# ZechengLi19/CIM

Measured on AMD Instinct MI355X. Metric: images/sec training step (ResNet-50 VOC, ~1k proposals/img) at 1/2/4/8 GPU, higher is better.
Workload: dtype fp32

## Files before the change

cim_amd/csrc/conv1x1.hip:

```cpp
#include "common.h"
#include "../../include/cim_hip.h"

#ifndef CIM_BODY_PRIO_LEVEL
#define CIM_BODY_PRIO_LEVEL 3
#endif
#if CIM_BODY_PRIO_LEVEL > 0
#define CIM_BODY_PRIO() __builtin_amdgcn_s_setprio(CIM_BODY_PRIO_LEVEL)
#else
#define CIM_BODY_PRIO()
#endif
namespace {

#ifndef CIM_SMALL_BK
#define CIM_SMALL_BK 32
#endif
#ifndef CIM_SMALL_ABL
#define CIM_SMALL_ABL 0
#endif
constexpr int SBM = 64, SBN = 64, SBK = CIM_SMALL_BK;
constexpr int SLD = 68;
typedef float f32x16 __attribute__((ext_vector_type(16)));
typedef float f32x4u __attribute__((ext_vector_type(4), aligned(4)));
__device__ __forceinline__ float4 ld4(const float* p) {
    const f32x4u v = *reinterpret_cast<const f32x4u*>(p);
// ... 193 lines not shown
#define SM_GLOAD(RA, RB, S)                                                                                        \
    {                                                                                                              \
        _Pragma("unroll") for (int i = 0; i < PA; ++i) asm volatile("" : "+v"(RA[i].x), "+v"(RA[i].y), "+v"(RA[i].z), "+v"(RA[i].w)); \
        _Pragma("unroll") for (int i = 0; i < PB; ++i) asm volatile("" : "+v"(RB[i].x), "+v"(RB[i].y), "+v"(RB[i].z), "+v"(RB[i].w)); \
    }
#else
#define SM_GLOAD(RA, RB, S)                                                                                        \
    {                                                                                                              \
        _Pragma("unroll") for (int i = 0; i < PA; ++i) RA[i] = bld4(RA_, oa[i] + (unsigned)(S) * sa);               \
        _Pragma("unroll") for (int i = 0; i < PB; ++i) RB[i] = bld4(RB_, ob[i] + (unsigned)(S) * sb);               \
    }
#endif
#define SM_PUT(RA, RB, BUF, S)                                                                                     \
    {                                                                                                              \
        _Pragma("unroll") for (int i = 0; i < PA; ++i)                                                             \
            tile_store<AM, SBM>(As[BUF], tile_ktail<AM, SBM>(RA[i], g.K, kbeg + (S) * SBK, tid + i * NT), tid + i * NT);     \
        _Pragma("unroll") for (int i = 0; i < PB; ++i)                                                             \
            tile_store<!BKc, BNT>(Bs[BUF], tile_ktail<!BKc, BNT>(RB[i], g.K, kbeg + (S) * SBK, tid + i * NT), tid + i * NT); \
    }
#define SM_MMA(BUF)                                                                                                \
    {                                                                                                              \
        const float* __restrict__ a = As[BUF] + (lane >> 5) * SLD + wm * 32 + (lane & 31);                         \
        const float* __restrict__ b = Bs[BUF] + (lane >> 5) * SLD + wn * 32 + (lane & 31);                         \
        float av[SBK / 2], bv[SBK / 2];                                                                            \
        _Pragma("unroll") for (int t = 0; t < SBK / 2; ++t) { av[t] = a[2 * t * SLD]; bv[t] = b[2 * t * SLD]; }    \
        _Pragma("unroll") for (int t = 0; t < (CIM_SMALL_ABL == 1 ? 1 : SBK / 2); ++t)                             \
            acc = __builtin_amdgcn_mfma_f32_32x32x2f32(av[t], bv[t], acc, 0, 0, 0);                                \
        asm volatile("" : "+a"(acc));       \
    }
    if (kbeg < kend) {
        const int nslab = (kend - kbeg + SBK - 1) / SBK;
        const int last = nslab - 1;
        SM_GLOAD(ra0, rb0, 0)
        SM_GLOAD(ra1, rb1, min(1, last))
        SM_PUT(ra0, rb0, 0, 0)
        asm volatile("" : "+a"(acc));
        __syncthreads();
        for (int s = 0; s < nslab; s += 2) {
            SM_GLOAD(ra0, rb0, min(s + 2, last))
            SM_MMA(0)
            if (s + 1 < nslab) SM_PUT(ra1, rb1, 1, s + 1)
            __syncthreads();
            if (s + 1 >= nslab) break;
            SM_GLOAD(ra1, rb1, min(s + 3, last))
            SM_MMA(1)
            if (s + 2 < nslab) SM_PUT(ra0, rb0, 0, s + 2)
            __syncthreads();
        }
    }
#undef SM_GLOAD
#undef SM_PUT
#undef SM_MMA

    small_epilogue(g, acc, m0 + wm * 32, n0 + wn * 32, lane, split, ColIdentity{g.N});
}

__device__ __forceinline__ float splitk_sum(const float* __restrict__ ws, size_t i, size_t mn, int splits) {
    float v = ws[i];
    for (int k0 = 1; k0 < splits; k0 += 8) {
        float p[8];
#pragma unroll
        for (int j = 0; j < 8; ++j) p[j] = k0 + j < splits ? ws[(size_t)(k0 + j) * mn + i] : 0.0f;
#pragma unroll
        for (int j = 0; j < 8; ++j)
            if (k0 + j < splits) v += p[j];
    }
    return v;
}
__global__ __launch_bounds__(256) void small_splitk_reduce_kernel(const SmallArgs g) {
    CIM_BODY_PRIO();
    const size_t i = (size_t)blockIdx.x * 256 + threadIdx.x;
    const size_t mn = (size_t)g.M * g.N;
    if (i >= mn) return;
    small_finish(g, (int)(i / g.N), (int)(i % g.N), splitk_sum(g.ws, i, mn, g.splits));
}
__global__ __launch_bounds__(256) void small_splitk_reduce4_kernel(const SmallArgs g) {
    CIM_BODY_PRIO();
    const size_t q = (size_t)blockIdx.x * 256 + threadIdx.x;
    const size_t mn = (size_t)g.M * g.N;
    const size_t i = q * 4;
    if (i >= mn) return;
    float4 v = *reinterpret_cast<const float4*>(g.ws + i);
    for (int k0 = 1; k0 < g.splits; k0 += 4) {
        float4 p[4];
#pragma unroll
        for (int j = 0; j < 4; ++j)
            p[j] = k0 + j < g.splits ? *reinterpret_cast<const float4*>(g.ws + (size_t)(k0 + j) * mn + i) : make_float4(0.f, 0.f, 0.f, 0.f);
#pragma unroll
        for (int j = 0; j < 4; ++j)
            if (k0 + j < g.splits) { v.x += p[j].x; v.y += p[j].y; v.z += p[j].z; v.w += p[j].w; }
    }
    int row = (int)(i / g.N), col = (int)(i - (size_t)row * g.N);
    const float s[4] = {v.x, v.y, v.z, v.w};
    float y[4], s1 = 0.0f, s2 = 0.0f;
#pragma unroll
    for (int j = 0; j < 4; ++j) {
        y[j] = small_value(g, row, col, s[j], s1, s2);
        if (++col == g.N) { col = 0; ++row; }
    }
    if (g.Xraw) *reinterpret_cast<float4*>(g.Xraw + i) = v;
    *reinterpret_cast<float4*>(g.C + i) = make_float4(y[0], y[1], y[2], y[3]);
}

__global__ __launch_bounds__(256) void small_splitk_reduce_rows_kernel(const SmallArgs g) {
    CIM_BODY_PRIO();
    const int col = blockIdx.x * 256 + threadIdx.x, row = blockIdx.y;
    const size_t mn = (size_t)g.M * g.N;
    float s1 = 0.0f, s2 = 0.0f;
    if (col < g.N) {
        const size_t i = (size_t)row * g.N + col;
        small_finish(g, row, col, splitk_sum(g.ws, i, mn, g.splits), s1, s2);
    }
    small_put_part(g, row, col >> 5, threadIdx.x & 63, s1, s2);
}

struct BnPartTable { cim_bn_part_desc d[24]; int first[25]; int n; };
__global__ __launch_bounds__(256) void bn_part_finish_kernel(const BnPartTable t) {
    CIM_BODY_PRIO();
    __shared__ float sh[2][8][32];
    int e = 0;
    while (e + 1 < t.n && (int)blockIdx.x >= t.first[e + 1]) ++e;
    const cim_bn_part_desc& d = t.d[e];
    const int C = d.channels, parts = d.parts, total = d.images * d.parts;
    const int c = ((int)blockIdx.x - t.first[e]) * 32 + (threadIdx.x & 31), grp = threadIdx.x >> 5;
    float t1 = 0.0f, t2 = 0.0f;
    if (c < C) {
        for (int i0 = grp; i0 < total; i0 += 32) {
            float a[4], b[4];
#pragma unroll
            for (int j = 0; j < 4; ++j) {
                const int i = i0 + 8 * j;
                const int img = i / parts, p = i - img * parts;
                const float* q = d.part + ((size_t)img * 2 * parts + p) * C + c;
                a[j] = i < total ? q[0] : 0.0f;
                b[j] = i < total ? q[(size_t)parts * C] : 0.0f;
            }
#pragma unroll
            for (int j = 0; j < 4; ++j) { t1 += a[j]; t2 += b[j]; }
        }
    }
    sh[0][grp][threadIdx.x & 31] = t1;
    sh[1][grp][threadIdx.x & 31] = t2;
    __syncthreads();
    if (grp == 0 && c < C) {
        float a1 = 0.0f, a2 = 0.0f;
#pragma unroll
        for (int k = 0; k < 8; ++k) { a1 += sh[0][k][threadIdx.x]; a2 += sh[1][k][threadIdx.x]; }
        if (d.dbeta) d.dbeta[c] = a1;
        if (d.dgamma) d.dgamma[c] = a2 * rsqrtf(d.var[c] + d.eps);
    }
}

enum { CONV_FWD = 0, CONV_DX = 1, CONV_DW = 2 };
struct ConvGeom { int H, W, Ho, Wo, stride, cin, cout; float inv_w; int dil; };

#ifndef CIM_CONV3_BK
#define CIM_CONV3_BK 32
#endif
constexpr int CBK = CIM_CONV3_BK;
template <int MODE, int KS = 3>
__global__ __launch_bounds__(256) void conv3x3_small_kernel(const SmallArgs g, const ConvGeom c) {
    CIM_BODY_PRIO();
    constexpr int TAPS = KS * KS;
    constexpr int NT = 256, PA = SBM * (CBK / 4) / NT, PB = SBN * (CBK / 4) / NT;
    extern __shared__ __attribute__((aligned(16))) float c3_smem[];
    float (*As)[CBK * SLD] = reinterpret_cast<float (*)[CBK * SLD]>(c3_smem);
    float (*Bs)[CBK * SLD] = reinterpret_cast<float (*)[CBK * SLD]>(c3_smem + 2 * CBK * SLD);
    const int tid = threadIdx.x, lane = tid & 63, wave = tid >> 6;
    const int wm = wave >> 1, wn = wave & 1;
    const int tiles_n = (g.N + SBN - 1) / SBN;
    const int m0 = (blockIdx.x / tiles_n) * SBM, n0 = (blockIdx.x % tiles_n) * SBN;
    const int split = blockIdx.y;
    const int kper = ((g.K + g.splits - 1) / g.splits + CBK - 1) / CBK * CBK;
    const int kbeg = split * kper, kend = min(g.K, kbeg + kper);

    const rsrc_t RA_ = make_rsrc(g.A, tile_extent(MODE == CONV_DX, g.M, g.K, g.lda));
    const rsrc_t RB_ = make_rsrc(g.B, (long long)(MODE == CONV_DX ? c.cout * c.Ho * c.Wo : c.cin * c.H * c.W));
    const int hw_src = MODE == CONV_DX ? c.Ho * c.Wo : c.H * c.W;
    int py[PB][4], px[PB][4];
    int boff[PB], bdy[PB], bdx[PB];
#pragma unroll
    for (int i = 0; i < PB; ++i) {
        const int p = tid + i * NT;
        if (MODE == CONV_DW) {
            const int n = n0 + p % SBN;
            const int ch = n / TAPS, tap = n - ch * TAPS;
            boff[i] = n < g.N ? ch * hw_src : -1;
            bdy[i] = (tap / KS - KS / 2) * c.dil;
            bdx[i] = (tap - (tap / KS) * KS - KS / 2) * c.dil;
        } else {
            const int wrow = (MODE == CONV_DX) ? c.W : c.Wo;
#pragma unroll
            for (int j = 0; j < 4; ++j) {
                const int n = n0 + (p % 16) * 4 + j;
                const int y = (int)(((float)n + 0.5f) * c.inv_w);
                py[i][j] = n < g.N ? y : -(1 << 20);
                px[i][j] = n - y * wrow;
            }
        }
    }
    unsigned oa[PA];
#pragma unroll
    for (int i = 0; i < PA; ++i) oa[i] = tile_off<MODE == CONV_DX, SBM>(g.lda, m0, kbeg, tid + i * NT);
    const unsigned sa = (MODE == CONV_DX ? (unsigned)g.lda * CBK : (unsigned)CBK) * 4u;

    auto load_b = [&](int k0, float4 (&rb)[PB]) {
#pragma unroll
        for (int i = 0; i < PB; ++i) {
            const int p = tid + i * NT;
            unsigned off[4];
            if (MODE == CONV_DW) {
                const int k = k0 + (p / SBN) * 4;
#pragma unroll
                for (int j = 0; j < 4; ++j) {
                    const int po = k + j;
                    const int yo = (int)(((float)po + 0.5f) * c.inv_w), xo = po - yo * c.Wo;
                    const int yi = yo * c.stride + bdy[i], xi = xo * c.stride + bdx[i];
                    const bool ok = boff[i] >= 0 && po < g.K && (unsigned)yi < (unsigned)c.H && (unsigned)xi < (unsigned)c.W;
                    off[j] = ok ? (unsigned)(boff[i] + yi * c.W + xi) * 4u : OOB;
                }
            } else {
                const int k = k0 + p / 16;
                const int ch = k / TAPS, tap = k - ch * TAPS;
                const int dy = (tap / KS - KS / 2) * c.dil, dx = (tap - (tap / KS) * KS - KS / 2) * c.dil;
                const int base = ch * hw_src;
#pragma unroll
                for (int j = 0; j < 4; ++j) {
                    if (MODE == CONV_DX) {
                        const int ty = py[i][j] - dy, tx = px[i][j] - dx;
                        const int yo = c.stride == 2 ? ty >> 1 : ty, xo = c.stride == 2 ? tx >> 1 : tx;
                        const bool ok = ty >= 0 && tx >= 0 && yo < c.Ho && xo < c.Wo && !(c.stride == 2 && ((ty | tx) & 1));
                        off[j] = ok ? (unsigned)(base + yo * c.Wo + xo) * 4u : OOB;
                    } else {
                        const int yi = py[i][j] * c.stride + dy, xi = px[i][j] * c.stride + dx;
                        const bool ok = (unsigned)yi < (unsigned)c.H && (unsigned)xi < (unsigned)c.W;
                        off[j] = ok ? (unsigned)(base + yi * c.W + xi) * 4u : OOB;
                    }
                }
            }
#if CIM_SMALL_ABL == 3
            asm volatile("" : "+v"(rb[i].x), "+v"(rb[i].y), "+v"(rb[i].z), "+v"(rb[i].w) : "v"(off[0]), "v"(off[1]), "v"(off[2]), "v"(off[3]));
#elif CIM_SMALL_ABL == 5
            rb[i] = make_float4(bld1(RB_, (unsigned)(p * 16 + k0 * 64)), bld1(RB_, (unsigned)(p * 16 + k0 * 64 + 4)),
                                bld1(RB_, (unsigned)(p * 16 + k0 * 64 + 8)), bld1(RB_, (unsigned)(p * 16 + k0 * 64 + 12)));
#else
            rb[i] = make_float4(bld1(RB_, off[0]), bld1(RB_, off[1]), bld1(RB_, off[2]), bld1(RB_, off[3]));
#endif
        }
    };
    auto load_a = [&](int s, float4 (&ra)[PA]) {
#pragma unroll
        for (int i = 0; i < PA; ++i)
            ra[i] = bld4(RA_, oa[i] + (unsigned)s * sa);
    };

    f32x16 acc;
#pragma unroll
    for (int i = 0; i < 16; ++i) acc[i] = 0.0f;
    float4 ra0[PA], rb0[PB], ra1[PA], rb1[PB];
#define C3_PUT(RA, RB, BUF, S)                                                                                      \
    {                                                                                                               \
        _Pragma("unroll") for (int i = 0; i < PA; ++i)                                                              \
            tile_store<MODE == CONV_DX, SBM>(As[BUF], tile_ktail<MODE == CONV_DX, SBM>(RA[i], g.K, kbeg + (S) * CBK, tid + i * NT), tid + i * NT); \
        _Pragma("unroll") for (int i = 0; i < PB; ++i) tile_store<MODE != CONV_DW, SBN>(Bs[BUF], RB[i], tid + i * NT); \
    }
#define C3_MMA(BUF)                                                                                                 \
    {                                                                                                               \
        const float* __restrict__ a = As[BUF] + (lane >> 5) * SLD + wm * 32 + (lane & 31);                          \
        const float* __restrict__ b = Bs[BUF] + (lane >> 5) * SLD + wn * 32 + (lane & 31);                          \
        float av[CBK / 2], bv[CBK / 2];                                                                             \
        _Pragma("unroll") for (int t = 0; t < CBK / 2; ++t) { av[t] = a[2 * t * SLD]; bv[t] = b[2 * t * SLD]; }     \
        _Pragma("unroll") for (int t = 0; t < (CIM_SMALL_ABL == 1 ? 1 : CBK / 2); ++t)                              \
            acc = __builtin_amdgcn_mfma_f32_32x32x2f32(av[t], bv[t], acc, 0, 0, 0);                                 \
        asm volatile("" : "+a"(acc));                                                                               \
    }
    if (kbeg < kend) {
        const int nslab = (kend - kbeg + CBK - 1) / CBK;
        const int last = nslab - 1;
        load_a(0, ra0); load_b(kbeg, rb0);
        load_a(min(1, last), ra1); load_b(kbeg + min(1, last) * CBK, rb1);
        C3_PUT(ra0, rb0, 0, 0)
        asm volatile("" : "+a"(acc));
        __syncthreads();
        for (int s = 0; s < nslab; s += 2) {
            load_a(min(s + 2, last), ra0); load_b(kbeg + min(s + 2, last) * CBK, rb0);
            C3_MMA(0)
            if (s + 1 < nslab) C3_PUT(ra1, rb1, 1, s + 1)
            __syncthreads();
            if (s + 1 >= nslab) break;
            load_a(min(s + 3, last), ra1); load_b(kbeg + min(s + 3, last) * CBK, rb1);
            C3_MMA(1)
            if (s + 2 < nslab) C3_PUT(ra0, rb0, 0, s + 2)
            __syncthreads();
        }
    }
#undef C3_PUT
#undef C3_MMA
    small_epilogue(g, acc, m0 + wm * 32, n0 + wn * 32, lane, split, ColIdentity{g.N});
}

struct Dx2Geom { int H, W, Ho, Wo, cin, cout; int first[5]; int tiles_n[4]; int group0[4]; };

__global__ __launch_bounds__(256) void conv3x3_dx2_kernel(const SmallArgs g, const Dx2Geom c) {
    CIM_BODY_PRIO();
    constexpr int NT = 256, PA = SBM * (CBK / 4) / NT, PB = SBN * (CBK / 4) / NT;
    extern __shared__ __attribute__((aligned(16))) float d2_smem[];
    float (*As)[CBK * SLD] = reinterpret_cast<float (*)[CBK * SLD]>(d2_smem);
    float (*Bs)[CBK * SLD] = reinterpret_cast<float (*)[CBK * SLD]>(d2_smem + 2 * CBK * SLD);
    const int tid = threadIdx.x, lane = tid & 63, wave = tid >> 6;
    const int wm = wave >> 1, wn = wave & 1;
    int cls = 0;
    while (cls < 3 && (int)blockIdx.x >= c.first[cls + 1]) ++cls;
    const int py = cls >> 1, px = cls & 1;
    const int Wc = (c.W - px + 1) >> 1, Nc = ((c.H - py + 1) >> 1) * Wc;
    const int local = (int)blockIdx.x - c.first[cls], tn = c.tiles_n[cls];
    const int m0 = (local / tn) * SBM, n0 = (local % tn) * SBN;
    const int nx = px ? 2 : 1, lgT = py + px, T = 1 << lgT;
    const int K = c.cout << lgT;
    const int nslab = (K + CBK - 1) / CBK;
    const int how = c.Ho * c.Wo;
    const rsrc_t RA_ = make_rsrc(g.A, tile_extent(true, g.M, 9 * c.cout, g.lda));
    const rsrc_t RB_ = make_rsrc(g.B, (long long)c.cout * how);
    int yc[PB][4], xc[PB][4];
#pragma unroll
    for (int i = 0; i < PB; ++i) {
        const int p = tid + i * NT;
#pragma unroll
        for (int j = 0; j < 4; ++j) {
            const int nc = n0 + (p % 16) * 4 + j;
            const int y = nc / Wc;
            yc[i][j] = nc < Nc ? y : -(1 << 20);
            xc[i][j] = nc - y * Wc;
        }
    }
    auto tap_of = [&](int j, int& tap, int& oy, int& ox) {
        const int jy = j / nx, jx = j - jy * nx;
        const int ky = py ? 2 * jy : 1, kx = px ? 2 * jx : 1;
        tap = ky * 3 + kx;
        oy = (py && jy == 0) ? 1 : 0;
        ox = (px && jx == 0) ? 1 : 0;
    };
    auto load_a = [&](int k0, float4 (&ra)[PA]) {
#pragma unroll
        for (int i = 0; i < PA; ++i) {
            const int p = tid + i * NT;
            const int k = k0 + p / (SBM / 4), r = m0 + (p % (SBM / 4)) * 4;
            const int co = k >> lgT;
            int tap, oy, ox;
            tap_of(k & (T - 1), tap, oy, ox);
            ra[i] = bld4(RA_, co < c.cout ? ((unsigned)(co * 9 + tap) * g.lda + r) * 4u : OOB);
        }
    };
    auto load_b = [&](int k0, float4 (&rb)[PB]) {
#pragma unroll
        for (int i = 0; i < PB; ++i) {
            const int p = tid + i * NT;
            const int k = k0 + p / 16;
            const int co = k >> lgT;
            int tap, oy, ox;
            tap_of(k & (T - 1), tap, oy, ox);
            const int base = co * how;
            unsigned off[4];
#pragma unroll
            for (int j = 0; j < 4; ++j) {
                const int yo = yc[i][j] + oy, xo = xc[i][j] + ox;
                const bool ok = co < c.cout && yo >= 0 && yo < c.Ho && xo < c.Wo;
                off[j] = ok ? (unsigned)(base + yo * c.Wo + xo) * 4u : OOB;
            }
            rb[i] = make_float4(bld1(RB_, off[0]), bld1(RB_, off[1]), bld1(RB_, off[2]), bld1(RB_, off[3]));
        }
    };
    f32x16 acc;
#pragma unroll
    for (int i = 0; i < 16; ++i) acc[i] = 0.0f;
    float4 ra0[PA], rb0[PB], ra1[PA], rb1[PB];
#define D2_PUT(RA, RB, BUF)                                                                                         \
    {                                                                                                               \
        _Pragma("unroll") for (int i = 0; i < PA; ++i) tile_store<true, SBM>(As[BUF], RA[i], tid + i * NT);          \
        _Pragma("unroll") for (int i = 0; i < PB; ++i) tile_store<true, SBN>(Bs[BUF], RB[i], tid + i * NT);          \
    }
#define D2_MMA(BUF)                                                                                                 \
    {                                                                                                               \
        const float* __restrict__ a = As[BUF] + (lane >> 5) * SLD + wm * 32 + (lane & 31);                          \
        const float* __restrict__ b = Bs[BUF] + (lane >> 5) * SLD + wn * 32 + (lane & 31);                          \
        float av[CBK / 2], bv[CBK / 2];                                                                             \
        _Pragma("unroll") for (int t = 0; t < CBK / 2; ++t) { av[t] = a[2 * t * SLD]; bv[t] = b[2 * t * SLD]; }     \
        _Pragma("unroll") for (int t = 0; t < CBK / 2; ++t)                                                         \
            acc = __builtin_amdgcn_mfma_f32_32x32x2f32(av[t], bv[t], acc, 0, 0, 0);                                 \
        asm volatile("" : "+a"(acc));                                                                               \
    }
    {
        const int last = nslab - 1;
        load_a(0, ra0); load_b(0, rb0);
        load_a(min(1, last) * CBK, ra1); load_b(min(1, last) * CBK, rb1);
        D2_PUT(ra0, rb0, 0)
        asm volatile("" : "+a"(acc));
        __syncthreads();
        for (int s = 0; s < nslab; s += 2) {
            load_a(min(s + 2, last) * CBK, ra0); load_b(min(s + 2, last) * CBK, rb0);
            D2_MMA(0)
            if (s + 1 < nslab) D2_PUT(ra1, rb1, 1)
            __syncthreads();
            if (s + 1 >= nslab) break;
            load_a(min(s + 3, last) * CBK, ra1); load_b(min(s + 3, last) * CBK, rb1);
            D2_MMA(1)
            if (s + 2 < nslab) D2_PUT(ra0, rb0, 0)
            __syncthreads();
        }
    }
#undef D2_PUT
#undef D2_MMA
    small_epilogue(g, acc, m0 + wm * 32, n0 + wn * 32, lane, 0, ColParity{Wc, c.W, py, px, Nc, c.group0[cls]});
}

__global__ __launch_bounds__(256) void conv3x3_wt_kernel(const float* __restrict__ w, float* __restrict__ wt, int cin) {
    extern __shared__ float wt_s[];
    const int co = blockIdx.x, n = cin * 9;
    for (int i = threadIdx.x; i < n; i += 256) wt_s[i] = w[(size_t)co * n + i];
    __syncthreads();
    for (int i = threadIdx.x; i < n; i += 256) {
        const int tap = i / cin, ci = i - tap * cin;
        wt[(size_t)co * n + i] = wt_s[ci * 9 + tap];
    }
}

struct WtTable { cim_wt_desc d[16]; int first[17]; int n; };
__global__ __launch_bounds__(256) void conv3x3_wt_multi_kernel(const WtTable t) {
    extern __shared__ float wt_s[];
    int e = 0;
    while (e + 1 < t.n && (int)blockIdx.x >= t.first[e + 1]) ++e;
    const int co = blockIdx.x - t.first[e], cin = t.d[e].cin, n = cin * 9;
    const float* __restrict__ w = t.d[e].w;
    float* __restrict__ wt = t.d[e].wt;
    for (int i = threadIdx.x; i < n; i += 256) wt_s[i] = w[(size_t)co * n + i];
    __syncthreads();
    for (int i = threadIdx.x; i < n; i += 256) {
        const int tap = i / cin, ci = i - tap * cin;
        wt[(size_t)co * n + i] = wt_s[ci * 9 + tap];
    }
}

SmallArgs small_args(const float* A, const float* B, float* C, int M, int N, int K, int lda, int ldb, int ldc, int splits, float* ws,
                     const InputBn* in_bn, float* x_raw = nullptr, const float* gamma = nullptr, const float* beta = nullptr,
                     const float* mean = nullptr, const float* var = nullptr, float eps = 0.f, const float* residual = nullptr, int relu = 0) {
    SmallArgs g{};
    g.A = A; g.B = B; g.C = C; g.Xraw = x_raw;
    g.gamma = gamma; g.beta = beta; g.mean = mean; g.var = var; g.res = residual; g.eps = eps;
    g.M = M; g.N = N; g.K = K; g.lda = lda; g.ldb = ldb; g.ldc = ldc;
    g.relu = relu; g.bn = gamma != nullptr;
    g.splits = splits; g.ws = ws;
    if (in_bn) {
        g.mask = in_bn->y; g.mgamma = in_bn->gamma; g.mvar = in_bn->var; g.meps = in_bn->eps;
        g.mxr = in_bn->xr; g.mmean = in_bn->mean; g.mpart = in_bn->part; g.mparts = (N + 31) / 32;
    }
    return g;
}
template <class Kernel, class... Args>
int launch_lds(Kernel kern, dim3 grid, size_t lds, hipStream_t st, const Args&... args) {
    if (lds > 48 * 1024) {
        hipError_t e = hipFuncSetAttribute(reinterpret_cast<const void*>(kern), hipFuncAttributeMaxDynamicSharedMemorySize, (int)lds);
        if (e != hipSuccess) return (int)e;
    }
    hipLaunchKernelGGL(kern, grid, dim3(256), lds, st, args...);
    return 0;
}
static void launch_splitk_reduce(const SmallArgs& g, hipStream_t st) {
    if (g.mpart) {
        hipLaunchKernelGGL(small_splitk_reduce_rows_kernel, dim3((unsigned)((g.N + 255) / 256), (unsigned)g.M), dim3(256), 0, st, g);
    } else {
        const size_t n = (size_t)g.M * g.N;
        if (n >= (1u << 19) && g.ldc == g.N && n % 4 == 0 && (((size_t)g.ws | (size_t)g.C | (size_t)g.Xraw) & 15) == 0)
            hipLaunchKernelGGL(small_splitk_reduce4_kernel, dim3((unsigned)((n / 4 + 255) / 256)), dim3(256), 0, st, g);
        else
            hipLaunchKernelGGL(small_splitk_reduce_kernel, dim3((unsigned)((n + 255) / 256)), dim3(256), 0, st, g);
    }
}

template <bool AM, bool BKc>
static void launch_small(const SmallArgs& g, int splits, hipStream_t st, bool narrow) {
    const long long tm = (g.M + SBM - 1) / SBM;
    if (narrow)
        hipLaunchKernelGGL((gemm_small_kernel<AM, BKc, 1>), dim3((unsigned)(tm * ((g.N + 31) / 32)), (unsigned)splits), dim3(128), 0, st, g);
    else
        hipLaunchKernelGGL((gemm_small_kernel<AM, BKc, 2>), dim3((unsigned)(tm * ((g.N + 63) / 64)), (unsigned)splits), dim3(256), 0, st, g);
}

}

extern "C" int cim_gemm_small_splits(int M, int N, int K) {
    const long long tiles = (long long)((M + SBM - 1) / SBM) * ((N + SBN - 1) / SBN);
#ifndef CIM_SMALL_WGS
#define CIM_SMALL_WGS 512
#endif
#ifndef CIM_SMALL_MINSLABS
#define CIM_SMALL_MINSLABS 4
#endif
    constexpr int min_k = CIM_SMALL_MINSLABS * SBK, want = CIM_SMALL_WGS;
    int s = 1;
    while (tiles * s < want && K / (s * 2) >= min_k && s < 64) s *= 2;
    return s;
}

static int gemm_small_impl(const float* A, const float* B, float* C, int M, int N, int K, int lda, int ldb, int ldc,
                           int a_mcontig, int b_kcontig, float* x_raw, const float* gamma, const float* beta,
                           const float* mean, const float* var, float eps, const float* residual, int relu, int splits,
                           float* workspace, void* stream, const InputBn* in_bn, int res_w = 0) {
    CIM_CHECK_ARG(res_w == 0 || (residual && res_w > 0 && N % res_w == 0 && ldc == N));
    CIM_CHECK_ARG(A && B && C && M > 0 && N > 0 && K > 0 && lda > 0 && ldb > 0 && ldc >= N && splits >= 1);
    CIM_CHECK_ARG((gamma == nullptr) == (beta == nullptr) && (gamma == nullptr) == (mean == nullptr) && (gamma == nullptr) == (var == nullptr));
    CIM_CHECK_ARG(splits == 1 || workspace);
    SmallArgs g = small_args(A, B, C, M, N, K, lda, ldb, ldc, splits, workspace, in_bn, x_raw, gamma, beta, mean, var, eps, residual, relu);
    g.a_mcontig = a_mcontig; g.b_kcontig = b_kcontig;
    g.res_w = res_w;
    if (res_w) { g.res_ws = (res_w + 1) / 2; g.res_hw = ((N / res_w + 1) / 2) * g.res_ws; }
    const long long tiles = (long long)((M + SBM - 1) / SBM) * ((N + SBN - 1) / SBN);
    CIM_CHECK_ARG(tiles * 2 < (1ll << 31) && splits <= 65535 && M <= 65535);
    CIM_CHECK_ARG(tile_extent(a_mcontig != 0, M, K, lda) < (1ll << 29) && tile_extent(b_kcontig == 0, N, K, ldb) < (1ll << 29));
    const bool narrow = tiles * splits < 128;
    hipStream_t st = cim::as_stream(stream);
    if (a_mcontig) {
        if (b_kcontig) launch_small<true, true>(g, splits, st, narrow); else launch_small<true, false>(g, splits, st, narrow);
    } else {
        if (b_kcontig) launch_small<false, true>(g, splits, st, narrow); else launch_small<false, false>(g, splits, st, narrow);
    }
    if (splits > 1) launch_splitk_reduce(g, st);
    CIM_CHECK_LAUNCH();
    return 0;
}

extern "C" int cim_gemm_small_f32(const float* A, const float* B, float* C, int M, int N, int K, int lda, int ldb, int ldc,
                                  int a_mcontig, int b_kcontig, float* x_raw, const float* gamma, const float* beta,
                                  const float* mean, const float* var, float eps, const float* residual, int relu, int splits,
                                  float* workspace, void* stream) {
    return gemm_small_impl(A, B, C, M, N, K, lda, ldb, ldc, a_mcontig, b_kcontig, x_raw, gamma, beta, mean, var, eps, residual, relu,
                           splits, workspace, stream, nullptr);
}

extern "C" int cim_linear_bias_f32(const float* X, const float* W, const float* bias, float* Y, int M, int N, int K, int splits,
                                   float* workspace, void* stream) {
    CIM_CHECK_ARG(X && W && Y && M > 0 && N > 0 && K > 0 && splits >= 1 && splits <= 65535 && (splits == 1 || workspace));
    SmallArgs g = small_args(X, W, Y, M, N, K, K, K, N, splits, workspace, nullptr);
    g.b_kcontig = 1; g.colbias = bias;
    hipStream_t st = cim::as_stream(stream);
    launch_small<false, true>(g, splits, st, false);
    if (splits > 1) {
        const size_t n = (size_t)M * N;
        hipLaunchKernelGGL(small_splitk_reduce_kernel, dim3((unsigned)((n + 255) / 256)), dim3(256), 0, st, g);
    }
    CIM_CHECK_LAUNCH();
    return 0;
}

extern "C" long long cim_conv1x1_bwd_workspace(int B, int cin, int cout, int hw) {
    const long long dx = (long long)cim_gemm_small_splits(cin, hw, cout) * cin * hw;
    const long long dw = (long long)cim_gemm_small_splits(cout, cin, hw) * cout * cin + (B > 1 ? (long long)cout * cin : 0);
    const long long dconv = (long long)B * cout * hw;
    return (long long)sizeof(float) * (dconv + dx + dw);
}

namespace {
struct ForkJoin {
    hipStream_t main, side;
    hipEvent_t ev_fork, ev_join;
    bool on;
    ForkJoin(hipStream_t m, hipStream_t s, void* fork_event, void* join_event, bool want)
        : main(m), side(s), ev_fork(static_cast<hipEvent_t>(fork_event)), ev_join(static_cast<hipEvent_t>(join_event)),
          on(want && s != nullptr && s != m) {}
    hipStream_t fork() {
        if (!on) return main;
        (void)hipEventRecord(ev_fork, main);
        (void)hipStreamWaitEvent(side, ev_fork, 0);
        return side;
    }
    void join() {
        if (!on) return;
        (void)hipEventRecord(ev_join, side);
        (void)hipStreamWaitEvent(main, ev_join, 0);
    }
};

__global__ __launch_bounds__(256) void small_axpy_kernel(float* __restrict__ y, const float* __restrict__ x, size_t n) {
    const size_t i = (size_t)blockIdx.x * 256 + threadIdx.x;
    if (i < n) y[i] += x[i];
}
template <class Product>
int dw_over_images(int B, float* dw, float* ws_dw, int sp, size_t n, hipStream_t st, Product product) {
    for (int b = 0; b < B && dw; ++b) {
        float* out = b == 0 ? dw : ws_dw + (size_t)sp * n;
        const int rc = product(b, out);
        if (rc) return rc;
        if (b) hipLaunchKernelGGL(small_axpy_kernel, dim3((unsigned)((n + 255) / 256)), dim3(256), 0, st, dw, out, n);
    }
    return 0;
}
}

extern "C" int cim_conv1x1_bn_act_bwd(const float* dy, const float* y, const float* x_raw, const float* x, const float* w,
                                      const float* gamma, const float* mean, const float* var, float eps, int relu,
                                      float* dres, float* dgamma, float* dbeta, float* dx, float* dw, int B, int cin, int cout,
                                      int hw, float* workspace, void* stream, void* side_stream, void* fork_event, void* join_event, int join,
                                      int dy_is_dconv, const float* in_gamma, const float* in_var, float in_eps,
                                      const float* in_xr, const float* in_mean, float* in_part, const float* dx_add, int dx_add_w) {
    CIM_CHECK_ARG(dx_add_w == 0 || (dx_add != nullptr && dx_add_w > 0 && hw % dx_add_w == 0));
    CIM_CHECK_ARG(side_stream == nullptr || side_stream == stream || (fork_event != nullptr && (!join || join_event != nullptr)));
    const size_t add_bs = dx_add_w ? (size_t)cin * ((hw / dx_add_w + 1) / 2) * ((dx_add_w + 1) / 2) : (size_t)cin * hw;
    CIM_CHECK_ARG(dy && x_raw && x && w && gamma && mean && var && workspace && B > 0 && cin > 0 && cout > 0 && hw > 0);
    CIM_CHECK_ARG(dx_add == nullptr || (dx != nullptr && in_gamma == nullptr));
    CIM_CHECK_ARG((y != nullptr || !relu) && ((dgamma == nullptr) == (dbeta == nullptr)));
    CIM_CHECK_ARG(!dy_is_dconv || (dres == nullptr && dgamma == nullptr));
    CIM_CHECK_ARG((in_gamma == nullptr) == (in_var == nullptr));
    CIM_CHECK_ARG(in_part == nullptr || (in_gamma && in_xr && in_mean));
    float* dconv = dy_is_dconv ? const_cast<float*>(dy) : workspace;
    float* ws_dx = workspace + (size_t)B * cout * hw;
    float* ws_dw = ws_dx + (size_t)cim_gemm_small_splits(cin, hw, cout) * cin * hw;
    int rc = dy_is_dconv ? 0 : cim_bn_act_bwd(dy, y, x_raw, gamma, mean, var, eps, dconv, dres, dgamma, dbeta, B, cout, hw, relu, stream);
    if (rc) return rc;
    ForkJoin fj(cim::as_stream(stream), cim::as_stream(side_stream), fork_event, join_event, dx && dw);
    hipStream_t st_dw = fj.fork();
    const int sp = cim_gemm_small_splits(cout, cin, hw);
    rc = dw_over_images(B, dw, ws_dw, sp, (size_t)cout * cin, st_dw, [&](int b, float* out) {
        return cim_gemm_small_f32(dconv + (size_t)b * cout * hw, x + (size_t)b * cin * hw, out, cout, cin, hw, hw, hw, cin, 0, 1,
                                  nullptr, nullptr, nullptr, nullptr, nullptr, 0.f, nullptr, 0, sp, ws_dw, st_dw);
    });
    if (rc) return rc;
    for (int b = 0; b < B && dx; ++b) {
        const InputBn ib{x + (size_t)b * cin * hw, in_gamma, in_var, in_eps, in_xr ? in_xr + (size_t)b * cin * hw : nullptr, in_mean,
                         in_part ? in_part + (size_t)b * 2 * ((hw + 31) / 32) * cin : nullptr};
        rc = gemm_small_impl(w, dconv + (size_t)b * cout * hw, dx + (size_t)b * cin * hw, cin, hw, cout, cin, hw, hw, 1, 0,
                             nullptr, nullptr, nullptr, nullptr, nullptr, 0.f, dx_add ? dx_add + (size_t)b * add_bs : nullptr, 0,
                             cim_gemm_small_splits(cin, hw, cout), ws_dx, stream, in_gamma ? &ib : nullptr, dx_add_w);
        if (rc) return rc;
    }
    if (join) fj.join();
    CIM_CHECK_LAUNCH();
    return 0;
}

namespace {
int conv3x3_launch(int mode, const float* A, const float* B, float* C, int M, int N, int K, int lda, int ldc, const ConvGeom& c,
                   float* x_raw, const float* gamma, const float* beta, const float* mean, const float* var, float eps,
                   const float* residual, int relu, int splits, float* ws, hipStream_t st, int ksize = 3, const InputBn* in_bn = nullptr) {
    SmallArgs g = small_args(A, B, C, M, N, K, lda, 0, ldc, splits, ws, in_bn, x_raw, gamma, beta, mean, var, eps, residual, relu);
    g.b_kcontig = mode == CONV_DW;
    const dim3 grid((unsigned)(((M + SBM - 1) / SBM) * ((N + SBN - 1) / SBN)), (unsigned)splits);
    auto kern = ksize == 7 ? conv3x3_small_kernel<CONV_FWD, 7>
                : mode == CONV_FWD ? conv3x3_small_kernel<CONV_FWD> : mode == CONV_DX ? conv3x3_small_kernel<CONV_DX> : conv3x3_small_kernel<CONV_DW>;
    const int rc = launch_lds(kern, grid, sizeof(float) * 4 * CBK * SLD, st, g, c);
    if (rc) return rc;
    if (splits > 1) launch_splitk_reduce(g, st);
    return 0;
}
ConvGeom conv_geom(int cin, int cout, int H, int W, int stride, int mode, int dil = 1) {
    ConvGeom c;
    c.H = H; c.W = W; c.stride = stride; c.cin = cin; c.cout = cout; c.dil = dil;
    c.Ho = (H - 1) / stride + 1; c.Wo = (W - 1) / stride + 1;
    c.inv_w = 1.0f / (float)(mode == CONV_DX ? W : c.Wo);
    return c;
}
}

#define CONV3_ARGS_OK(CIN_MULT)                                                                                      \
    CIM_CHECK_ARG(cin > 0 && cout > 0 && H > 0 && W > 0 && (stride == 1 || stride == 2) && W <= 4096 &&               \
                  dilation >= 1 && dilation <= 8 && (dilation == 1 || stride == 1) &&                                 \
                  (long long)H * W < (1ll << 20) && (long long)cin * H * W < (1ll << 29) && (long long)cout * H * W < (1ll << 29) && \
                  (long long)cin * cout * 9 < (1ll << 29) && cin % (CIN_MULT) == 0)

extern "C" int cim_conv3x3_nchw_splits(int cin, int cout, int H, int W, int stride) {
    const int Ho = (H - 1) / stride + 1, Wo = (W - 1) / stride + 1;
    return cim_gemm_small_splits(cout, Ho * Wo, 9 * cin);
}

extern "C" int cim_conv3x3_nchw_f32(const float* x, const float* w, float* y, int cin, int cout, int H, int W, int stride,
                               int dilation, float* x_raw, const float* gamma, const float* beta, const float* mean, const float* var,
                               float eps, const float* residual, int relu, int splits, float* workspace, void* stream) {
    CIM_CHECK_ARG(x && w && y && splits >= 1 && splits <= 65535 && (splits == 1 || workspace));
    CONV3_ARGS_OK(1);
    CIM_CHECK_ARG((gamma == nullptr) == (beta == nullptr) && (gamma == nullptr) == (mean == nullptr) && (gamma == nullptr) == (var == nullptr));
    const ConvGeom c = conv_geom(cin, cout, H, W, stride, CONV_FWD, dilation);
    conv3x3_launch(CONV_FWD, w, x, y, cout, c.Ho * c.Wo, 9 * cin, 9 * cin, c.Ho * c.Wo, c, x_raw, gamma, beta, mean, var, eps,
                   residual, relu, splits, workspace, cim::as_stream(stream));
    CIM_CHECK_LAUNCH();
    return 0;
}

extern "C" int cim_conv7x7_nchw_f32(const float* x, const float* w, float* y, int cin, int cout, int H, int W, int stride,
                                    const float* gamma, const float* beta, const float* mean, const float* var, float eps,
                                    int relu, void* stream) {
    CIM_CHECK_ARG(x && w && y && cin > 0 && cout > 0 && H > 0 && W > 0 && (stride == 1 || stride == 2) && W <= 4096);
    CIM_CHECK_ARG((long long)H * W < (1ll << 20) && (long long)cin * H * W < (1ll << 29) && (long long)cout * H * W < (1ll << 29));
    CIM_CHECK_ARG((gamma == nullptr) == (beta == nullptr) && (gamma == nullptr) == (mean == nullptr) && (gamma == nullptr) == (var == nullptr));
    const ConvGeom c = conv_geom(cin, cout, H, W, stride, CONV_FWD);
    conv3x3_launch(CONV_FWD, w, x, y, cout, c.Ho * c.Wo, 49 * cin, 49 * cin, c.Ho * c.Wo, c, nullptr, gamma, beta, mean, var, eps,
                   nullptr, relu, 1, nullptr, cim::as_stream(stream), 7);
    CIM_CHECK_LAUNCH();
    return 0;
}

namespace {
Dx2Geom dx2_geom(int cin, int cout, int H, int W) {
    Dx2Geom c{};
    c.H = H; c.W = W; c.Ho = (H - 1) / 2 + 1; c.Wo = (W - 1) / 2 + 1; c.cin = cin; c.cout = cout;
    const int tiles_m = (cin + SBM - 1) / SBM;
    int first = 0, group = 0;
    for (int cls = 0; cls < 4; ++cls) {
        const int py = cls >> 1, px = cls & 1;
        const int nc = ((H - py + 1) / 2) * ((W - px + 1) / 2);
        c.first[cls] = first;
        c.tiles_n[cls] = (nc + SBN - 1) / SBN;
        c.group0[cls] = group;
        first += tiles_m * c.tiles_n[cls];
        group += 2 * c.tiles_n[cls];
    }
    c.first[4] = first;
    return c;
}
}

extern "C" int cim_conv3x3_dx_parts(int H, int W, int stride) {
    if (stride != 2) return (H * W + 31) / 32;
    int parts = 0;
    for (int cls = 0; cls < 4; ++cls) parts += 2 * ((((H - (cls >> 1) + 1) / 2) * ((W - (cls & 1) + 1) / 2) + SBN - 1) / SBN);
    return parts;
}

extern "C" long long cim_conv3x3_nchw_bwd_workspace(int B, int cin, int cout, int H, int W, int stride) {
    const int Ho = (H - 1) / stride + 1, Wo = (W - 1) / stride + 1;
    const long long dx = (long long)cim_gemm_small_splits(cin, H * W, 9 * cout) * cin * H * W;
    const long long dw = (long long)cim_gemm_small_splits(cout, 9 * cin, Ho * Wo) * cout * cin * 9 + (B > 1 ? (long long)cout * cin * 9 : 0);
    const long long dconv = (long long)B * cout * Ho * Wo;
    return (long long)sizeof(float) * (dconv + (long long)cout * cin * 9 + dx + dw);
}

extern "C" int cim_bn_part_finish(const cim_bn_part_desc* descs, int n, void* stream) {
    CIM_CHECK_ARG(descs && n > 0);
    hipStream_t st = cim::as_stream(stream);
    for (int base = 0; base < n; base += 24) {
        BnPartTable t{};
        t.n = n - base < 24 ? n - base : 24;
        int total = 0;
        for (int i = 0; i < t.n; ++i) {
            const cim_bn_part_desc& d = descs[base + i];
            CIM_CHECK_ARG(d.part && d.var && (d.dgamma || d.dbeta) && d.images > 0 && d.parts > 0 && d.channels > 0);
            t.d[i] = d;
            t.first[i] = total;
            total += (d.channels + 31) / 32;
        }
        t.first[t.n] = total;
        hipLaunchKernelGGL(bn_part_finish_kernel, dim3((unsigned)total), dim3(256), 0, st, t);
    }
    CIM_CHECK_LAUNCH();
    return 0;
}

extern "C" int cim_conv3x3_wt_multi(const cim_wt_desc* descs, int n, void* stream) {
    CIM_CHECK_ARG(descs && n > 0);
    hipStream_t st = cim::as_stream(stream);
    for (int base = 0; base < n; base += 16) {
        WtTable t{};
        t.n = n - base < 16 ? n - base : 16;
        int total = 0, max_cin = 0;
        for (int i = 0; i < t.n; ++i) {
            const cim_wt_desc& d = descs[base + i];
            CIM_CHECK_ARG(d.w && d.wt && d.cin > 0 && d.cout > 0 && (size_t)d.cin * 9 * sizeof(float) <= 64 * 1024);
            t.d[i] = d;
            t.first[i] = total;
            total += d.cout;
            max_cin = d.cin > max_cin ? d.cin : max_cin;
        }
        t.first[t.n] = total;
        const int rc = launch_lds(conv3x3_wt_multi_kernel, dim3((unsigned)total), sizeof(float) * max_cin * 9, st, t);
        if (rc) return rc;
    }
    CIM_CHECK_LAUNCH();
    return 0;
}

extern "C" int cim_conv3x3_nchw_bn_act_bwd(const float* dy, const float* y, const float* x_raw, const float* x, const float* w,
                                      const float* gamma, const float* mean, const float* var, float eps, int relu,
                                      float* dres, float* dgamma, float* dbeta, float* dx, float* dw, int B, int cin, int cout,
                                      int H, int W, int stride, int dilation, float* workspace, void* stream, void* side_stream,
                                      void* fork_event, void* join_event, int join, int dy_is_dconv, const float* in_gamma, const float* in_var, float in_eps,
                                      const float* in_xr, const float* in_mean, float* in_part, const float* wt_ready) {
    CIM_CHECK_ARG(dy && x_raw && x && w && gamma && mean && var && workspace && B > 0);
    CIM_CHECK_ARG(side_stream == nullptr || side_stream == stream || (fork_event != nullptr && (!join || join_event != nullptr)));
    CONV3_ARGS_OK(4);
    CIM_CHECK_ARG((y != nullptr || !relu) && ((dgamma == nullptr) == (dbeta == nullptr)) && cout % 4 == 0);
    CIM_CHECK_ARG(!dy_is_dconv || (dres == nullptr && dgamma == nullptr));
    CIM_CHECK_ARG((in_gamma == nullptr) == (in_var == nullptr));
    CIM_CHECK_ARG(in_part == nullptr || (in_gamma && in_xr && in_mean));
    const ConvGeom cx = conv_geom(cin, cout, H, W, stride, CONV_DX, dilation), cw = conv_geom(cin, cout, H, W, stride, CONV_DW, dilation);
    const int hwo = cx.Ho * cx.Wo, hw = H * W;
    hipStream_t st = cim::as_stream(stream);
    float* dconv = dy_is_dconv ? const_cast<float*>(dy) : workspace;
    float* wt_own = workspace + (size_t)B * cout * hwo;
    const float* wt = wt_ready ? wt_ready : wt_own;
    float* ws_dx = wt_own + (size_t)cout * cin * 9;
    float* ws_dw = ws_dx + (size_t)cim_gemm_small_splits(cin, hw, 9 * cout) * cin * hw;
    CIM_CHECK_ARG((size_t)cin * 9 * sizeof(float) <= 64 * 1024);
    int rc = dy_is_dconv ? 0 : cim_bn_act_bwd(dy, y, x_raw, gamma, mean, var, eps, dconv, dres, dgamma, dbeta, B, cout, hwo, relu, stream);
    if (rc) return rc;
    ForkJoin fj(st, cim::as_stream(side_stream), fork_event, join_event, dx && dw);
    hipStream_t st_dw = fj.fork();
    const int sp = cim_gemm_small_splits(cout, 9 * cin, hwo);
    rc = dw_over_images(B, dw, ws_dw, sp, (size_t)cout * cin * 9, st_dw, [&](int b, float* out) {
        return conv3x3_launch(CONV_DW, dconv + (size_t)b * cout * hwo, x + (size_t)b * cin * hw, out, cout, 9 * cin, hwo, hwo, 9 * cin, cw,
                              nullptr, nullptr, nullptr, nullptr, nullptr, 0.f, nullptr, 0, sp, ws_dw, st_dw);
    });
    if (rc) return rc;
    if (dx && !wt_ready) hipLaunchKernelGGL(conv3x3_wt_kernel, dim3(cout), dim3(256), sizeof(float) * cin * 9, st, w, wt_own, cin);
// ... 22 lines not shown
```

Before: 75.71.

## Precompute tap validity masks and gather offsets in implicit-GEMM conv kernels

Reworks address generation in the 3x3/7x7 implicit-GEMM kernels so each thread keeps one output pixel column and a bitmask of valid kernel rows and columns. Per-load bounds checks then become a single mask test plus an add. The B tile mapping changes so the k index is uniform per wave, and the DW path replaces float division with a magic-number multiply. The stride-2 deconv kernel now precomputes per-slab base offsets and validity selectors. The change also drops stride-2 support from the DX conv3x3 path (now guarded by an argument check) and changes the B tile store layout, which risks correctness if other code relied on the old layout.

```diff
diff --git a/cim_amd/csrc/conv1x1.hip b/cim_amd/csrc/conv1x1.hip
--- a/cim_amd/csrc/conv1x1.hip
+++ b/cim_amd/csrc/conv1x1.hip
@@ -369,7 +369,7 @@
 }
 
 enum { CONV_FWD = 0, CONV_DX = 1, CONV_DW = 2 };
-struct ConvGeom { int H, W, Ho, Wo, stride, cin, cout; float inv_w; int dil; };
+struct ConvGeom { int H, W, Ho, Wo, stride, cin, cout; float inv_w; int dil; unsigned mag_wo; };
 
 #ifndef CIM_CONV3_BK
 #define CIM_CONV3_BK 32
@@ -394,26 +394,32 @@
     const rsrc_t RA_ = make_rsrc(g.A, tile_extent(MODE == CONV_DX, g.M, g.K, g.lda));
     const rsrc_t RB_ = make_rsrc(g.B, (long long)(MODE == CONV_DX ? c.cout * c.Ho * c.Wo : c.cin * c.H * c.W));
     const int hw_src = MODE == CONV_DX ? c.Ho * c.Wo : c.H * c.W;
-    int py[PB][4], px[PB][4];
-    int boff[PB], bdy[PB], bdx[PB];
-#pragma unroll
-    for (int i = 0; i < PB; ++i) {
-        const int p = tid + i * NT;
+    static_assert(NT % SBN == 0 && NT / SBN * PB * 4 == CBK && KS <= 8, "piece mapping");
+    const unsigned hw4 = (unsigned)hw_src * 4u;
+    const int wsrc = MODE == CONV_DX ? c.Wo : c.W, hsrc = MODE == CONV_DX ? c.Ho : c.H;
+    const int tstep_y = (MODE == CONV_DX ? -4 : 4) * c.dil * wsrc, tstep_x = (MODE == CONV_DX ? -4 : 4) * c.dil;
+    int pbase = 0; unsigned pmask = 0;
+    int wboff = 0, wdy = 0, wdx = 0;
+    {
+        const int n = n0 + tid % SBN;
         if (MODE == CONV_DW) {
-            const int n = n0 + p % SBN;
             const int ch = n / TAPS, tap = n - ch * TAPS;
-            boff[i] = n < g.N ? ch * hw_src : -1;
-            bdy[i] = (tap / KS - KS / 2) * c.dil;
-            bdx[i] = (tap - (tap / KS) * KS - KS / 2) * c.dil;
+            const int dy = (tap / KS - KS / 2) * c.dil;
+            wdx = (tap - (tap / KS) * KS - KS / 2) * c.dil;
+            wboff = (ch * hw_src + dy * c.W + wdx) * 4;
+            wdy = n < g.N ? dy : (1 << 20);
         } else {
             const int wrow = (MODE == CONV_DX) ? c.W : c.Wo;
-#pragma unroll
-            for (int j = 0; j < 4; ++j) {
-                const int n = n0 + (p % 16) * 4 + j;
-                const int y = (int)(((float)n + 0.5f) * c.inv_w);
-                py[i][j] = n < g.N ? y : -(1 << 20);
-                px[i][j] = n - y * wrow;
-            }
+            const int pad = (KS / 2) * c.dil, sgn = MODE == CONV_DX ? -1 : 1;
+            const int y = (int)(((float)n + 0.5f) * c.inv_w), x = n - y * wrow;
+            const int y0 = MODE == CONV_DX ? y + pad : y * c.stride - pad, x0 = MODE == CONV_DX ? x + pad : x * c.stride - pad;
+            unsigned m = 0;
+#pragma unroll
+            for (int t = 0; t < KS; ++t)
+                m |= ((unsigned)((unsigned)(y0 + sgn * t * c.dil) < (unsigned)hsrc) << t) |
+                     ((unsigned)((unsigned)(x0 + sgn * t * c.dil) < (unsigned)wsrc) << (8 + t));
+            pmask = n < g.N ? m : 0u;
+            pbase = (y0 * wsrc + x0) * 4;
         }
     }
     unsigned oa[PA];
@@ -421,43 +427,38 @@
     for (int i = 0; i < PA; ++i) oa[i] = tile_off<MODE == CONV_DX, SBM>(g.lda, m0, kbeg, tid + i * NT);
     const unsigned sa = (MODE == CONV_DX ? (unsigned)g.lda * CBK : (unsigned)CBK) * 4u;
 
+    const int wave_u = __builtin_amdgcn_readfirstlane(wave);
+    const unsigned wo_is_1 = c.mag_wo ? 0u : ~0u;
     auto load_b = [&](int k0, float4 (&rb)[PB]) {
 #pragma unroll
         for (int i = 0; i < PB; ++i) {
-            const int p = tid + i * NT;
             unsigned off[4];
+            const int k = k0 + (wave_u + i * (NT / SBN)) * 4;
             if (MODE == CONV_DW) {
-                const int k = k0 + (p / SBN) * 4;
 #pragma unroll
                 for (int j = 0; j < 4; ++j) {
                     const int po = k + j;
-                    const int yo = (int)(((float)po + 0.5f) * c.inv_w), xo = po - yo * c.Wo;
-                    const int yi = yo * c.stride + bdy[i], xi = xo * c.stride + bdx[i];
-                    const bool ok = boff[i] >= 0 && po < g.K && (unsigned)yi < (unsigned)c.H && (unsigned)xi < (unsigned)c.W;
-                    off[j] = ok ? (unsigned)(boff[i] + yi * c.W + xi) * 4u : OOB;
+                    const int yo = (int)(__umulhi((unsigned)po, c.mag_wo) + ((unsigned)po & wo_is_1)), xo = po - yo * c.Wo;
+                    const int ys = po < g.K ? yo * c.stride : (1 << 20), xs = xo * c.stride;
+                    const bool ok = ((unsigned)(ys + wdy) < (unsigned)c.H) & ((unsigned)(xs + wdx) < (unsigned)c.W);
+                    const unsigned in = (unsigned)wboff + ((unsigned)ys * (unsigned)c.W + (unsigned)xs) * 4u;
+                    off[j] = ok ? in : OOB;
                 }
             } else {
-                const int k = k0 + p / 16;
-                const int ch = k / TAPS, tap = k - ch * TAPS;
-                const int dy = (tap / KS - KS / 2) * c.dil, dx = (tap - (tap / KS) * KS - KS / 2) * c.dil;
-                const int base = ch * hw_src;
 #pragma unroll
                 for (int j = 0; j < 4; ++j) {
-                    if (MODE == CONV_DX) {
-                        const int ty = py[i][j] - dy, tx = px[i][j] - dx;
-                        const int yo = c.stride == 2 ? ty >> 1 : ty, xo = c.stride == 2 ? tx >> 1 : tx;
-                        const bool ok = ty >= 0 && tx >= 0 && yo < c.Ho && xo < c.Wo && !(c.stride == 2 && ((ty | tx) & 1));
-                        off[j] = ok ? (unsigned)(base + yo * c.Wo + xo) * 4u : OOB;
-                    } else {
-                        const int yi = py[i][j] * c.stride + dy, xi = px[i][j] * c.stride + dx;
-                        const bool ok = (unsigned)yi < (unsigned)c.H && (unsigned)xi < (unsigned)c.W;
-                        off[j] = ok ? (unsigned)(base + yi * c.W + xi) * 4u : OOB;
-                    }
+                    const unsigned ch = (unsigned)(k + j) / TAPS, tap = (unsigned)(k + j) - ch * TAPS;
+                    const unsigned ky = tap / KS, kx = tap - ky * KS;
+                    const unsigned sel = (1u << ky) | (256u << kx);
+                    const unsigned toff = ch * hw4 + (unsigned)((int)ky * tstep_y + (int)kx * tstep_x);
+                    const unsigned in = toff + (unsigned)pbase;
+                    off[j] = (pmask & sel) == sel ? in : OOB;
                 }
             }
 #if CIM_SMALL_ABL == 3
             asm volatile("" : "+v"(rb[i].x), "+v"(rb[i].y), "+v"(rb[i].z), "+v"(rb[i].w) : "v"(off[0]), "v"(off[1]), "v"(off[2]), "v"(off[3]));
 #elif CIM_SMALL_ABL == 5
+            const int p = tid + i * NT;
             rb[i] = make_float4(bld1(RB_, (unsigned)(p * 16 + k0 * 64)), bld1(RB_, (unsigned)(p * 16 + k0 * 64 + 4)),
                                 bld1(RB_, (unsigned)(p * 16 + k0 * 64 + 8)), bld1(RB_, (unsigned)(p * 16 + k0 * 64 + 12)));
 #else
@@ -479,7 +480,7 @@
     {                                                                                                               \
         _Pragma("unroll") for (int i = 0; i < PA; ++i)                                                              \
             tile_store<MODE == CONV_DX, SBM>(As[BUF], tile_ktail<MODE == CONV_DX, SBM>(RA[i], g.K, kbeg + (S) * CBK, tid + i * NT), tid + i * NT); \
-        _Pragma("unroll") for (int i = 0; i < PB; ++i) tile_store<MODE != CONV_DW, SBN>(Bs[BUF], RB[i], tid + i * NT); \
+        _Pragma("unroll") for (int i = 0; i < PB; ++i) tile_store<false, SBN>(Bs[BUF], RB[i], tid + i * NT);         \
     }
 #define C3_MMA(BUF)                                                                                                 \
     {                                                                                                               \
@@ -538,18 +539,17 @@
     const int how = c.Ho * c.Wo;
     const rsrc_t RA_ = make_rsrc(g.A, tile_extent(true, g.M, 9 * c.cout, g.lda));
     const rsrc_t RB_ = make_rsrc(g.B, (long long)c.cout * how);
-    int yc[PB][4], xc[PB][4];
-#pragma unroll
-    for (int i = 0; i < PB; ++i) {
-        const int p = tid + i * NT;
-#pragma unroll
-        for (int j = 0; j < 4; ++j) {
-            const int nc = n0 + (p % 16) * 4 + j;
-            const int y = nc / Wc;
-            yc[i][j] = nc < Nc ? y : -(1 << 20);
-            xc[i][j] = nc - y * Wc;
-        }
-    }
+    static_assert(NT % 16 == 0 && CBK % 4 == 0, "gather state");
+    int lin[4]; unsigned vm[4];
+#pragma unroll
+    for (int j = 0; j < 4; ++j) {
+        const int nc = n0 + (tid % 16) * 4 + j;
+        const int y = nc / Wc, x = nc - y * Wc;
+        lin[j] = (y * c.Wo + x) * 4;
+        vm[j] = nc < Nc ? (unsigned)(y < c.Ho) | (unsigned)(y + 1 < c.Ho) << 1 | (unsigned)(x < c.Wo) << 2 | (unsigned)(x + 1 < c.Wo) << 3 : 0u;
+    }
+    unsigned oa[PA], ob[PB], bsel[PB];
+    const unsigned sa = (unsigned)(CBK >> lgT) * 9u * (unsigned)g.lda * 4u, sb = (unsigned)(CBK >> lgT) * (unsigned)how * 4u;
     auto tap_of = [&](int j, int& tap, int& oy, int& ox) {
         const int jy = j / nx, jx = j - jy * nx;
         const int ky = py ? 2 * jy : 1, kx = px ? 2 * jx : 1;
@@ -557,33 +557,33 @@
         oy = (py && jy == 0) ? 1 : 0;
         ox = (px && jx == 0) ? 1 : 0;
     };
-    auto load_a = [&](int k0, float4 (&ra)[PA]) {
-#pragma unroll
-        for (int i = 0; i < PA; ++i) {
-            const int p = tid + i * NT;
-            const int k = k0 + p / (SBM / 4), r = m0 + (p % (SBM / 4)) * 4;
-            const int co = k >> lgT;
-            int tap, oy, ox;
-            tap_of(k & (T - 1), tap, oy, ox);
-            ra[i] = bld4(RA_, co < c.cout ? ((unsigned)(co * 9 + tap) * g.lda + r) * 4u : OOB);
-        }
+#pragma unroll
+    for (int i = 0; i < PA; ++i) {
+        const int p = tid + i * NT;
+        const int k = p / (SBM / 4), r = m0 + (p % (SBM / 4)) * 4;
+        int tap, oy, ox;
+        tap_of(k & (T - 1), tap, oy, ox);
+        oa[i] = ((unsigned)((k >> lgT) * 9 + tap) * g.lda + r) * 4u;
+    }
+#pragma unroll
+    for (int i = 0; i < PB; ++i) {
+        const int k = (tid + i * NT) / 16;
+        int tap, oy, ox;
+        tap_of(k & (T - 1), tap, oy, ox);
+        ob[i] = (unsigned)((k >> lgT) * how + oy * c.Wo + ox) * 4u;
+        bsel[i] = (1u << oy) | (4u << ox);
+    }
+    auto load_a = [&](int s, float4 (&ra)[PA]) {
+#pragma unroll
+        for (int i = 0; i < PA; ++i) ra[i] = bld4(RA_, oa[i] + (unsigned)s * sa);
     };
-    auto load_b = [&](int k0, float4 (&rb)[PB]) {
+    auto load_b = [&](int s, float4 (&rb)[PB]) {
 #pragma unroll
         for (int i = 0; i < PB; ++i) {
-            const int p = tid + i * NT;
-            const int k = k0 + p / 16;
-            const int co = k >> lgT;
-            int tap, oy, ox;
-            tap_of(k & (T - 1), tap, oy, ox);
-            const int base = co * how;
+            const unsigned base = ob[i] + (unsigned)s * sb;
             unsigned off[4];
 #pragma unroll
-            for (int j = 0; j < 4; ++j) {
-                const int yo = yc[i][j] + oy, xo = xc[i][j] + ox;
-                const bool ok = co < c.cout && yo >= 0 && yo < c.Ho && xo < c.Wo;
-                off[j] = ok ? (unsigned)(base + yo * c.Wo + xo) * 4u : OOB;
-            }
+            for (int j = 0; j < 4; ++j) off[j] = (vm[j] & bsel[i]) == bsel[i] ? base + (unsigned)lin[j] : OOB;
             rb[i] = make_float4(bld1(RB_, off[0]), bld1(RB_, off[1]), bld1(RB_, off[2]), bld1(RB_, off[3]));
         }
     };
@@ -609,17 +609,17 @@
     {
         const int last = nslab - 1;
         load_a(0, ra0); load_b(0, rb0);
-        load_a(min(1, last) * CBK, ra1); load_b(min(1, last) * CBK, rb1);
+        load_a(min(1, last), ra1); load_b(min(1, last), rb1);
         D2_PUT(ra0, rb0, 0)
         asm volatile("" : "+a"(acc));
         __syncthreads();
         for (int s = 0; s < nslab; s += 2) {
-            load_a(min(s + 2, last) * CBK, ra0); load_b(min(s + 2, last) * CBK, rb0);
+            load_a(min(s + 2, last), ra0); load_b(min(s + 2, last), rb0);
             D2_MMA(0)
             if (s + 1 < nslab) D2_PUT(ra1, rb1, 1)
             __syncthreads();
             if (s + 1 >= nslab) break;
-            load_a(min(s + 3, last) * CBK, ra1); load_b(min(s + 3, last) * CBK, rb1);
+            load_a(min(s + 3, last), ra1); load_b(min(s + 3, last), rb1);
             D2_MMA(1)
             if (s + 2 < nslab) D2_PUT(ra0, rb0, 0)
             __syncthreads();
@@ -859,6 +859,7 @@
                    const float* residual, int relu, int splits, float* ws, hipStream_t st, int ksize = 3, const InputBn* in_bn = nullptr) {
     SmallArgs g = small_args(A, B, C, M, N, K, lda, 0, ldc, splits, ws, in_bn, x_raw, gamma, beta, mean, var, eps, residual, relu);
     g.b_kcontig = mode == CONV_DW;
+    CIM_CHECK_ARG(mode != CONV_DX || c.stride == 1);
     const dim3 grid((unsigned)(((M + SBM - 1) / SBM) * ((N + SBN - 1) / SBN)), (unsigned)splits);
     auto kern = ksize == 7 ? conv3x3_small_kernel<CONV_FWD, 7>
                 : mode == CONV_FWD ? conv3x3_small_kernel<CONV_FWD> : mode == CONV_DX ? conv3x3_small_kernel<CONV_DX> : conv3x3_small_kernel<CONV_DW>;
@@ -872,6 +873,7 @@
     c.H = H; c.W = W; c.stride = stride; c.cin = cin; c.cout = cout; c.dil = dil;
     c.Ho = (H - 1) / stride + 1; c.Wo = (W - 1) / stride + 1;
     c.inv_w = 1.0f / (float)(mode == CONV_DX ? W : c.Wo);
+    c.mag_wo = c.Wo > 1 ? (unsigned)(((1ull << 32) + c.Wo - 1) / c.Wo) : 0u;
     return c;
 }
 }
```

Result: no change. 76.51 (median of 4 runs) (+1.1%).
